# jwr1995/Conv-TasNet

Measured on AMD Instinct MI355X. Metric: utterances/sec (4s, 8kHz, 2-spk) fwd+bwd, higher is better.
Workload: dtype bf16; 1 GPU; paper config train step c2: N=256 L=20 B=256 H=512 P=3 X=8 R=4 gLN non-causal relu-mask, 2 spk, 4 s @ 8 kHz, fwd+PIT loss+bwd+clip+Adam; per_gpu_batch=32, global_batch=32, samples=32000, frames=3199, parallelism=dp1, hip_graph=False

## Files before the change

### conv-tasnet_amd/csrc/ctn_capi_codec.hip

```cpp
#include "ctn_capi_util.h"
#include "ctn_codec.h"

using namespace ctn;


static int codec_check(const ctn_codec_desc* d, bool need_b) {
  if (!d) return fail(CTN_ERR_ARG, "null descriptor");
  if (d->M < 1 || d->T < d->L || d->L < 2 || d->L > 32)
    return fail(CTN_ERR_UNSUPPORTED, "M=%d T=%d L=%d (need T >= L, 2 <= L <= 32)", d->M, d->T, d->L);
  const int S = d->L / 2;
  if (d->K != (d->T - d->L) / S + 1) return fail(CTN_ERR_ARG, "K=%d != (T-L)/(L/2)+1", d->K);
  if (d->Kp != ctn_padded_frames(d->K)) return fail(CTN_ERR_ARG, "Kp=%d != padded(K)", d->Kp);
  const int cg = d->N / 8;
  if (d->N % 8 || cg > 64 || (cg & (cg - 1)))
    return fail(CTN_ERR_UNSUPPORTED, "N=%d: need N/8 a power of two <= 64", d->N);
  if (need_b && (d->B % 8 || d->B < 8)) return fail(CTN_ERR_UNSUPPORTED, "B=%d must be a multiple of 8", d->B);
  if (d->C < 1 || d->C > 16) return fail(CTN_ERR_UNSUPPORTED, "C=%d outside 1..16", d->C);
  if (d->mask_type < 0 || d->mask_type > 2) return fail(CTN_ERR_ARG, "mask_type %d", d->mask_type);
  if (d->dtype != CTN_DTYPE_F32 && d->dtype != CTN_DTYPE_BF16) return fail(CTN_ERR_ARG, "dtype %d", d->dtype);
  return CTN_OK;
}

static CodecArgs codec_args(const ctn_codec_desc* d) {
  CodecArgs a{};
// ... 80 lines not shown
  if (!wb) return CTN_OK;
  const void* wbp = wb;
  if (dt == BF16) {
    CTN_HIP(launch_prep_weight(dt, wb, d->B, d->N, Ly.wbs, nullptr, s));
    wbp = Ly.wbs;
  }
  GemmRows g{};
  g.g = Rows{d->M, d->K, d->Kp}; g.Kred = d->N; g.Nout = d->B; g.norm = NORM_CLN;
  g.A = w_rows; g.lda = d->N;
  g.aop.kind = OP_NORM; g.aop.norm = NORM_CLN; g.aop.stats = a.cln_stats; g.aop.gamma = gamma0; g.aop.beta = beta0;
  g.W = wbp; g.ldw = d->N;
  g.epi = EPI_STORE; g.C = x0; g.ldc = d->B;
  CTN_HIP(launch_gemm_rows(dt, g, s));
  return CTN_OK;
}

extern "C" int ctn_encoder_backward(const ctn_codec_desc* d, const float* mixture, const float* U,
                                    const float* gamma0, const float* beta0, const float* wb, const void* w_rows,
                                    const float* cln_stats, const void* g_w_rows, const void* g_x0, float* gU,
                                    float* ggamma0, float* gbeta0, float* gwb, void* ws, size_t ws_bytes,
                                    void* stream) {
  int rc = codec_check(d, g_x0 != nullptr);
  if (rc) return rc;
  if (!mixture || !w_rows || !gU) return fail(CTN_ERR_ARG, "null pointer");
  if (g_x0 && (!wb || !gamma0 || !beta0 || !cln_stats || !ggamma0 || !gbeta0 || !gwb))
    return fail(CTN_ERR_ARG, "bottleneck backward needs wb/gamma0/beta0/stats and their gradient outputs");
  const EncLayout Ly = enc_layout(d, 1, ws);
  if (!ws || ws_bytes < Ly.bytes) return fail(CTN_ERR_WORKSPACE, "workspace %zu < %zu", ws_bytes, Ly.bytes);
  hipStream_t s = (hipStream_t)stream;
  const DType dt = d->dtype == CTN_DTYPE_BF16 ? BF16 : F32;
  const Rows rg{d->M, d->K, d->Kp};
  CodecArgs a = codec_args(d);
  a.mixture = mixture; a.U = U; a.w_rows = const_cast<void*>(w_rows);
  a.cln_stats = const_cast<float2*>(reinterpret_cast<const float2*>(cln_stats));
  a.gamma0 = gamma0; a.gwdec = g_w_rows; a.gpre = Ly.gpre; a.gpre_bf = Ly.gpre_bf;
  SlabBatch sb{};
  if (g_x0) {
    CTN_HIP(launch_prep_weight(dt, wb, d->B, d->N, nullptr, Ly.wbt, s));
    GemmRows g{};
    g.g = rg; g.Kred = d->B; g.Nout = d->N;
    g.A = g_x0; g.lda = d->B; g.W = Ly.wbt; g.ldw = d->B;
    g.epi = EPI_STORE; g.C = Ly.gcln; g.ldc = d->N;
    CTN_HIP(launch_gemm_rows(dt, g, s));
    GemmCols gc{};
    gc.g = rg; gc.P = d->B; gc.Q = d->N;
    gc.A = g_x0; gc.lda = d->B;
    gc.B = w_rows; gc.ldb = d->N;
    gc.bop.kind = OP_NORM; gc.bop.norm = NORM_CLN; gc.bop.stats = a.cln_stats; gc.bop.gamma = gamma0; gc.bop.beta = beta0;
    gc.Cpart = Ly.cpartB; gc.nchunks = Ly.chunksB;
    CTN_HIP(launch_gemm_cols(dt, gc, s));
    a.gcln = Ly.gcln;
    a.col_slab = Ly.colE;
    sb.d[sb.nd++] = SlabDesc{Ly.cpartB, gwb, Ly.chunksB, d->B * d->N, d->B * d->N};
    sb.d[sb.nd++] = SlabDesc{Ly.colE, ggamma0, Ly.rowblocks, d->N, 2 * d->N};
    sb.d[sb.nd++] = SlabDesc{Ly.colE + d->N, gbeta0, Ly.rowblocks, d->N, 2 * d->N};
  }
  CTN_HIP(launch_enc_bwd_rows(dt, a, s));
  const bool cols = Ly.gpre_bf != nullptr;
  if (cols) {
    a.Lp = Ly.Lp;
    CTN_HIP(launch_frames_bf16(a, mixture, 1, Ly.xfr, s));
    GemmCols gu = du_gemm(d, Ly.Lp);
    gu.A = Ly.gpre_bf; gu.lda = d->N; gu.B = Ly.xfr; gu.ldb = Ly.Lp;
    gu.Cpart = Ly.cpartU; gu.nchunks = Ly.chunksU;
    CTN_HIP(launch_gemm_cols(dt, gu, s));
    sb.d[sb.nd++] = SlabDesc{Ly.cpartU, Ly.Lp == d->L ? gU : Ly.tmpU, Ly.chunksU, d->N * Ly.Lp, d->N * Ly.Lp};
  } else {
    CodecArgs fo = a;
    fo.col_slab = Ly.slabU;
    CTN_HIP(launch_frame_outer(dt, 0, fo, s));
    sb.d[sb.nd++] = SlabDesc{Ly.slabU, gU, Ly.nU, d->N * d->L, d->N * d->L};
  }
  CTN_HIP(launch_slab_reduce(sb, Ly.srtmp, s));
  if (cols && Ly.Lp != d->L) CTN_HIP(launch_unpad_cols(Ly.tmpU, d->N, Ly.Lp, d->L, gU, s));
  return CTN_OK;
}

namespace {
bool dv_cols(const ctn_codec_desc* d) {
  const char* e = getenv("CTN_DV_COLS");
  if (e && atoi(e) == 0) return false;
  return codec_dec_mfma(d->dtype == CTN_DTYPE_BF16 ? BF16 : F32, codec_args(d));
}
GemmCols dv_gemm(const ctn_codec_desc* d, int Lp) {
  GemmCols g{};
  g.g = Rows{d->M, d->K * d->C, d->Kp * d->C};
  g.P = Lp; g.Q = d->N;
  return g;
}
struct DecLayout {
  void *wms, *wmt, *gscore, *srcb, *gfr;
  float *frames, *slabV, *cpartM, *cpartV, *srtmp;
  int nV, chunksM, chunksV, Lp;
  size_t bytes;
};
DecLayout dec_layout(const ctn_codec_desc* d, int backward, bool with_mask_conv, void* ws) {
  DecLayout L{};
  Carver c(ws);
  const size_t es = esize(d->dtype);
  const long rows = (long)d->M * d->Kp;
  const int CN = d->C * d->N;
  if (!backward) {
    if (with_mask_conv && d->dtype == CTN_DTYPE_BF16) L.wms = c.take<void>((size_t)CN * d->B * es);
    L.frames = c.take<float>((size_t)d->M * d->C * d->Kp * d->L * sizeof(float));
  } else {
    CodecArgs a = codec_args(d);
    if (dv_cols(d)) {
      L.Lp = (d->L + 7) & ~7;
      L.srcb = c.take<void>((size_t)rows * d->C * d->N * es);
      L.gfr = c.take<void>((size_t)rows * d->C * L.Lp * es);
      L.chunksV = gemm_cols_default_chunks(dv_gemm(d, L.Lp));
      L.cpartV = c.take<float>((size_t)L.chunksV * L.Lp * d->N * sizeof(float));
    } else {
      L.nV = frame_outer_chunks(a, d->C);
      L.slabV = c.take<float>((size_t)L.nV * d->N * d->L * sizeof(float));
    }
    if (with_mask_conv) {
      L.wmt = c.take<void>((size_t)CN * d->B * es);
      L.gscore = c.take<void>((size_t)rows * CN * es);
      GemmCols gc{};
      gc.g = Rows{d->M, d->K, d->Kp}; gc.P = CN; gc.Q = d->B;
      L.chunksM = gemm_cols_default_chunks(gc);
      L.cpartM = c.take<float>((size_t)L.chunksM * CN * d->B * sizeof(float));
    }
    L.srtmp = c.take<float>((sr_tmp(L.nV > L.chunksV ? L.nV : L.chunksV, (long)d->N * d->L) +
                             sr_tmp(L.chunksM, (long)CN * d->B)) * sizeof(float));
  }
  L.bytes = c.off + 256;
  return L;
}
}

extern "C" size_t ctn_decoder_workspace_bytes(const ctn_codec_desc* d, int backward) {
  if (codec_check(d, d && d->mask_type != CTN_MASK_IDENTITY) != CTN_OK) return 0;
  return dec_layout(d, backward, d->mask_type != CTN_MASK_IDENTITY, nullptr).bytes;
}

extern "C" int ctn_decoder_forward(const ctn_codec_desc* d, const void* x_last, const void* w_rows,
                                   const float* wm, const float* V, void* score, float* est, void* ws,
                                   size_t ws_bytes, void* stream) {
  int rc = codec_check(d, wm != nullptr);
  if (rc) return rc;
  if (!x_last || !w_rows || !V || !est) return fail(CTN_ERR_ARG, "null pointer");
  if ((wm == nullptr) != (d->mask_type == CTN_MASK_IDENTITY))
    return fail(CTN_ERR_ARG, "wm == NULL exactly when mask_type == CTN_MASK_IDENTITY (standalone Decoder)");
  if (wm && !score) return fail(CTN_ERR_ARG, "score output required with the mask conv");
  const DecLayout Ly = dec_layout(d, 0, wm != nullptr, ws);
  if (!ws || ws_bytes < Ly.bytes) return fail(CTN_ERR_WORKSPACE, "workspace %zu < %zu", ws_bytes, Ly.bytes);
  hipStream_t s = (hipStream_t)stream;
  const DType dt = d->dtype == CTN_DTYPE_BF16 ? BF16 : F32;
  const int CN = d->C * d->N;
  const void* sc = x_last;
  if (wm) {
    const void* wmp = wm;
    if (dt == BF16) {
      CTN_HIP(launch_prep_weight(dt, wm, CN, d->B, Ly.wms, nullptr, s));
      wmp = Ly.wms;
    }
    GemmRows g{};
    g.g = Rows{d->M, d->K, d->Kp}; g.Kred = d->B; g.Nout = CN;
    g.A = x_last; g.lda = d->B; g.W = wmp; g.ldw = d->B;
    g.epi = EPI_STORE; g.C = score; g.ldc = CN;
    CTN_HIP(launch_gemm_rows(dt, g, s));
    sc = score;
  }
  CodecArgs a = codec_args(d);
  a.w_rows = const_cast<void*>(w_rows); a.score = sc; a.V = V; a.frames = Ly.frames; a.est = est;
  CTN_HIP(launch_dec_fwd(dt, a, s));
  return CTN_OK;
}

extern "C" int ctn_decoder_backward(const ctn_codec_desc* d, const void* x_last, const void* w_rows,
                                    const float* wm, const float* V, const void* score, const float* g_est,
                                    void* g_x_last, void* g_w_rows, float* gwm, float* gV, void* ws,
                                    size_t ws_bytes, void* stream) {
  int rc = codec_check(d, wm != nullptr);
  if (rc) return rc;
  if (!x_last || !w_rows || !V || !g_est || !g_x_last || !g_w_rows || !gV) return fail(CTN_ERR_ARG, "null pointer");
  if ((wm == nullptr) != (d->mask_type == CTN_MASK_IDENTITY))
    return fail(CTN_ERR_ARG, "wm == NULL exactly when mask_type == CTN_MASK_IDENTITY (standalone Decoder)");
  if (wm && (!score || !gwm)) return fail(CTN_ERR_ARG, "score and gwm required with the mask conv");
  const DecLayout Ly = dec_layout(d, 1, wm != nullptr, ws);
  if (!ws || ws_bytes < Ly.bytes) return fail(CTN_ERR_WORKSPACE, "workspace %zu < %zu", ws_bytes, Ly.bytes);
  hipStream_t s = (hipStream_t)stream;
  const DType dt = d->dtype == CTN_DTYPE_BF16 ? BF16 : F32;
  const Rows rg{d->M, d->K, d->Kp};
  const int CN = d->C * d->N;
  CodecArgs a = codec_args(d);
  a.w_rows = const_cast<void*>(w_rows); a.score = wm ? score : x_last; a.V = V; a.gest = g_est;
  a.gscore = wm ? Ly.gscore : g_x_last; a.gwdec_out = g_w_rows;
  const bool cols = Ly.srcb != nullptr;
  if (cols) { a.src_out = Ly.srcb; a.gfr_out = Ly.gfr; a.Lp = Ly.Lp; }
  CTN_HIP(launch_dec_bwd(dt, a, s));
  SlabBatch sb{};
  if (cols) {
    CTN_HIP(launch_dec_gframes(a, s));
    GemmCols gv = dv_gemm(d, Ly.Lp);
    gv.A = Ly.gfr; gv.lda = Ly.Lp; gv.B = Ly.srcb; gv.ldb = d->N;
    gv.Cpart = Ly.cpartV; gv.nchunks = Ly.chunksV;
    CTN_HIP(launch_gemm_cols(dt, gv, s));
    sb.d[sb.nd++] = SlabDesc{Ly.cpartV, gV, Ly.chunksV, d->N * d->L, Ly.Lp * d->N};
  } else {
    CodecArgs fo = a;
    fo.col_slab = Ly.slabV;
    CTN_HIP(launch_frame_outer(dt, 1, fo, s));
    sb.d[sb.nd++] = SlabDesc{Ly.slabV, gV, Ly.nV, d->N * d->L, d->N * d->L};
  }
  if (wm) {
    CTN_HIP(launch_prep_weight(dt, wm, CN, d->B, nullptr, Ly.wmt, s));
    GemmRows g{};
    g.g = rg; g.Kred = CN; g.Nout = d->B;
    g.A = Ly.gscore; g.lda = CN; g.W = Ly.wmt; g.ldw = CN;
    g.epi = EPI_STORE; g.C = g_x_last; g.ldc = d->B;
    CTN_HIP(launch_gemm_rows(dt, g, s));
    GemmCols gc{};
    gc.g = rg; gc.P = CN; gc.Q = d->B;
    gc.A = Ly.gscore; gc.lda = CN; gc.B = x_last; gc.ldb = d->B;
    gc.Cpart = Ly.cpartM; gc.nchunks = Ly.chunksM;
    CTN_HIP(launch_gemm_cols(dt, gc, s));
    sb.d[sb.nd++] = SlabDesc{Ly.cpartM, gwm, Ly.chunksM, CN * d->B, CN * d->B};
  }
  CTN_HIP(launch_slab_reduce(sb, Ly.srtmp, s));
  return CTN_OK;
}
```

### conv-tasnet_amd/csrc/ctn_codec.h

```cpp
#pragma once
#include "ctn_kernels.h"

namespace ctn {

struct CodecArgs {
  int M, T, K, Kp, N, L, S, C;
  int mask_type;
  const float* mixture;
  const float* U;
  const float* V;
  void* w_rows;
  float2* cln_stats;
  const float* gamma0;
  const void* gcln;
  const void* gwdec;
  float* gpre;
  float* col_slab;
  const void* score;
  float* frames;
  float* est;
  const float* gest;
  void* gscore;
  void* gwdec_out;
  void* src_out = nullptr;
  void* gfr_out = nullptr;
  int Lp = 0;
  void* gpre_bf = nullptr;
};
bool codec_dec_mfma(DType dt, const CodecArgs& a);
hipError_t launch_dec_gframes(const CodecArgs& a, hipStream_t s);
hipError_t launch_frames_bf16(const CodecArgs& a, const float* sig, int C, void* out, hipStream_t s);
hipError_t launch_unpad_cols(const float* tmp, int N, int Lp, int L, float* out, hipStream_t s);

hipError_t launch_enc_fwd(DType dt, const CodecArgs& a, hipStream_t s);
hipError_t launch_enc_bwd_rows(DType dt, const CodecArgs& a, hipStream_t s);
int frame_outer_chunks(const CodecArgs& a, int C);
hipError_t launch_frame_outer(DType dt, int mode, const CodecArgs& a, hipStream_t s);
hipError_t launch_dec_fwd(DType dt, const CodecArgs& a, hipStream_t s);
hipError_t launch_dec_bwd(DType dt, const CodecArgs& a, hipStream_t s);

struct PitArgs {
  int M, C, T;
  const float* src;
  const float* est;
  const int64_t* lengths;
  double* slab;
  int chunks;
  float* max_snr;
  int64_t* best;
  float* coef;
  float* loss;
  const float* g_loss;
  const float* g_maxsnr;
  float* gest;
  float* est_inplace;
  float* reordered;
  double* msd;
  int nperm;
  int perms[24][4];
};
int pit_nv(int C);
hipError_t launch_pit_forward(const PitArgs& a, hipStream_t s);
hipError_t launch_pit_backward(const PitArgs& a, hipStream_t s);

}
```

### conv-tasnet_amd/csrc/ctn_codec.hip

```cpp
#include <stdlib.h>

#include "ctn_common.h"
#include "ctn_codec.h"

namespace ctn {

constexpr int EN_RPB = 128;

template <typename T>
__global__ __launch_bounds__(256) void enc_fwd_kernel(CodecArgs a) {
  extern __shared__ __attribute__((aligned(16))) float sm[];
  const int N = a.N, L = a.L, S = a.S, cg = N / 8;
  int nrl = 256 / cg;
  if (nrl > EN_RPB) nrl = EN_RPB;
  const int tid = threadIdx.x, c = tid % cg, rl = tid / cg;
  const bool act = rl < nrl;
  const int K = a.K, Kp = a.Kp;
  const int row0 = blockIdx.x * EN_RPB, m = row0 / Kp, k0 = row0 - m * Kp;
  float* Ut = sm;
  float* xs = sm + L * N;
  const int nsamp = (EN_RPB - 1) * S + L;
  for (int i = tid; i < L * N; i += 256) {
    const int l = i / N, n = i % N;
    Ut[i] = a.U[n * L + l];
// ... 363 lines not shown
    for (int c = 0; c < CM; ++c)
      if (c < C) mx = fmaxf(mx, x[c]);
#pragma unroll
    for (int c = 0; c < CM; ++c)
      if (c < C) {
        x[c] = __expf(x[c] - mx);
        den += x[c];
      }
#pragma unroll
    for (int c = 0; c < CM; ++c)
      if (c < C) x[c] /= den;
  } else if (mask_type == 0) {
#pragma unroll
    for (int c = 0; c < CM; ++c) x[c] = x[c] > 0.f ? x[c] : 0.f;
  }
}

template <int KBN, int CM>
__global__ __launch_bounds__(256) void dec_fwd_mfma_kernel(CodecArgs a) {
  constexpr int N = KBN * 32;
  __shared__ v4u bfrag[2 * KBN * 64];
  const int lane = threadIdx.x & 63, lg = lane >> 4, wv = threadIdx.x >> 6;
  const int L = a.L, C = a.C, K = a.K, Kp = a.Kp;
  for (int i = threadIdx.x; i < 2 * KBN * 64; i += 256) {
    const int ln = i & 63, kb = (i >> 6) % KBN, nb = i / (64 * KBN), l = nb * 16 + (ln & 15);
    float f[8] = {0, 0, 0, 0, 0, 0, 0, 0};
    if (l < L) Vec8<float>::load(a.V + (size_t)l * N + kb * 32 + 8 * (ln >> 4), f);
    bfrag[i] = pack_bf16x8v(f);
  }
  __syncthreads();
  const int lr = lane & 15;
  const bf16raw* w = reinterpret_cast<const bf16raw*>(a.w_rows);
  const bf16raw* sc = reinterpret_cast<const bf16raw*>(a.score);
  const long nblk = (long)a.M * Kp / 16;
  for (long blk = (long)blockIdx.x * DM_WAVES + wv; blk < nblk; blk += (long)gridDim.x * DM_WAVES) {
    const long r0 = blk * 16;
    const int m = (int)(r0 / Kp), k0 = (int)(r0 - (long)m * Kp);
    if (k0 >= K) continue;
    const long r = r0 + lr;
    f32x4_t acc[CM][2];
#pragma unroll
    for (int c = 0; c < CM; ++c) acc[c][0] = acc[c][1] = f32x4_t{0.f, 0.f, 0.f, 0.f};
#pragma unroll
    for (int kb = 0; kb < KBN; ++kb) {
      const int ch = kb * 32 + 8 * lg;
      float wf[8], sf[CM][8];
      unpack_bf16x8(ldg16(w + r * N + ch), wf);
#pragma unroll
      for (int c = 0; c < CM; ++c)
        if (c < C) unpack_bf16x8(ldg16(sc + r * (long)(C * N) + (long)c * N + ch), sf[c]);
#pragma unroll
      for (int e = 0; e < 8; ++e) {
        float x[CM];
#pragma unroll
        for (int c = 0; c < CM; ++c) x[c] = c < C ? sf[c][e] : 0.f;
        dm_act<CM>(a.mask_type, C, x);
#pragma unroll
        for (int c = 0; c < CM; ++c) sf[c][e] = wf[e] * x[c];
      }
#pragma unroll
      for (int c = 0; c < CM; ++c)
        if (c < C) {
          const bf16x8_t af = __builtin_bit_cast(bf16x8_t, pack_bf16x8v(sf[c]));
          const v4u b0 = bfrag[kb * 64 + lane], b1 = bfrag[(KBN + kb) * 64 + lane];
          acc[c][0] = __builtin_amdgcn_mfma_f32_16x16x32_bf16(af, __builtin_bit_cast(bf16x8_t, b0), acc[c][0], 0, 0, 0);
          acc[c][1] = __builtin_amdgcn_mfma_f32_16x16x32_bf16(af, __builtin_bit_cast(bf16x8_t, b1), acc[c][1], 0, 0, 0);
        }
    }
#pragma unroll
    for (int c = 0; c < CM; ++c)
      if (c < C)
#pragma unroll
        for (int nb = 0; nb < 2; ++nb) {
          const int l = nb * 16 + lr;
          if (l >= L) continue;
          float* f = a.frames + (((size_t)m * C + c) * Kp + k0) * L + l;
#pragma unroll
          for (int i = 0; i < 4; ++i)
            if (k0 + 4 * lg + i < K) f[(size_t)(4 * lg + i) * L] = acc[c][nb][i];
        }
  }
}

template <int NBN, int CM>
__global__ __launch_bounds__(256) void dec_bwd_mfma_kernel(CodecArgs a) {
  constexpr int N = NBN * 16;
  static_assert(NBN % 2 == 0, "two channel blocks per round");
  __shared__ v4u afrag[NBN * 64];
  constexpr int TS = 36;
  __shared__ __attribute__((aligned(16))) float gtile[DM_WAVES * CM * 16 * TS];
  const int lane = threadIdx.x & 63, lr = lane & 15, lg = lane >> 4, wv = threadIdx.x >> 6;
  const int L = a.L, C = a.C, S = a.S, K = a.K, Kp = a.Kp;
  for (int i = threadIdx.x; i < NBN * 64; i += 256) {
    const int ln = i & 63, nb = i >> 6;
    float f[8];
#pragma unroll
    for (int j = 0; j < 8; ++j) {
      const int l = 8 * (ln >> 4) + j;
      f[j] = l < L ? a.V[(size_t)l * N + nb * 16 + (ln & 15)] : 0.f;
    }
    afrag[i] = pack_bf16x8v(f);
  }
  __syncthreads();
  const bf16raw* w = reinterpret_cast<const bf16raw*>(a.w_rows);
  const bf16raw* sc = reinterpret_cast<const bf16raw*>(a.score);
  bf16raw* gsc = reinterpret_cast<bf16raw*>(a.gscore);
  bf16raw* gw = reinterpret_cast<bf16raw*>(a.gwdec_out);
  const long nblk = (long)a.M * Kp / 16;
  typedef uint32_t v2u __attribute__((ext_vector_type(2)));
  for (long blk = (long)blockIdx.x * DM_WAVES + wv; blk < nblk; blk += (long)gridDim.x * DM_WAVES) {
    const long r0 = blk * 16;
    const int m = (int)(r0 / Kp), k0 = (int)(r0 - (long)m * Kp);
    v4u gb[CM];
    {
      const int k = k0 + lr;
#pragma unroll
      for (int c = 0; c < CM; ++c) {
        float f[8] = {0, 0, 0, 0, 0, 0, 0, 0};
        if (c < C && k < K) {
          const float* g = a.gest + ((size_t)m * C + c) * a.T + (long)k * S;
#pragma unroll
          for (int j = 0; j < 8; ++j) {
            const int l = 8 * lg + j;
            if (l < L && (long)k * S + l < a.T) f[j] = g[l];
          }
        }
        gb[c] = pack_bf16x8v(f);
      }
    }
    float* tile = gtile + wv * (CM * 16 * TS);
    const int er = lane >> 2, en = 8 * (lane & 3);
#pragma unroll 1
    for (int nb = 0; nb < NBN; nb += 2) {
      const long r = r0 + er;
      const int n0 = nb * 16 + en;
      const v4u wraw = ldg16(w + r * N + n0);
      v4u sraw[CM];
#pragma unroll
      for (int c = 0; c < CM; ++c) sraw[c] = c < C ? ldg16(sc + r * (long)(C * N) + (long)c * N + n0) : v4u{0u, 0u, 0u, 0u};
#pragma unroll
      for (int h = 0; h < 2; ++h)
#pragma unroll
        for (int c = 0; c < CM; ++c)
          if (c < C) {
            const f32x4_t g = __builtin_amdgcn_mfma_f32_16x16x32_bf16(
                __builtin_bit_cast(bf16x8_t, afrag[(nb + h) * 64 + lane]), __builtin_bit_cast(bf16x8_t, gb[c]),
                f32x4_t{0.f, 0.f, 0.f, 0.f}, 0, 0, 0);
            *reinterpret_cast<float4*>(tile + (c * 16 + lr) * TS + h * 16 + 4 * lg) = float4{g[0], g[1], g[2], g[3]};
          }
      asm volatile("s_waitcnt lgkmcnt(0)" ::: "memory");
      float wf[8], sv[CM][8], gs[CM][8];
      unpack_bf16x8(wraw, wf);
#pragma unroll
      for (int c = 0; c < CM; ++c)
        if (c < C) {
          unpack_bf16x8(sraw[c], sv[c]);
          const float4 g0 = *reinterpret_cast<const float4*>(tile + (c * 16 + er) * TS + en);
          const float4 g1 = *reinterpret_cast<const float4*>(tile + (c * 16 + er) * TS + en + 4);
          gs[c][0] = g0.x; gs[c][1] = g0.y; gs[c][2] = g0.z; gs[c][3] = g0.w;
          gs[c][4] = g1.x; gs[c][5] = g1.y; gs[c][6] = g1.z; gs[c][7] = g1.w;
        }
      float gwv[8], go[CM][8], srcv[CM][8];
#pragma unroll
      for (int i = 0; i < 8; ++i) {
        float s[CM], act[CM];
#pragma unroll
        for (int c = 0; c < CM; ++c) {
          s[c] = c < C ? sv[c][i] : 0.f;
          act[c] = s[c];
        }
        dm_act<CM>(a.mask_type, C, act);
#pragma unroll
        for (int c = 0; c < CM; ++c) srcv[c][i] = wf[i] * act[c];
        float gwe = 0.f, dot = 0.f, ga[CM];
#pragma unroll
        for (int c = 0; c < CM; ++c) {
          ga[c] = 0.f;
          if (c < C) {
            gwe += gs[c][i] * act[c];
            ga[c] = gs[c][i] * wf[i];
            dot += ga[c] * act[c];
          }
        }
        gwv[i] = gwe;
#pragma unroll
        for (int c = 0; c < CM; ++c)
          if (c < C) {
            float g = ga[c];
            if (a.mask_type == 0 && !(s[c] > 0.f)) g = 0.f;
            if (a.mask_type == 1) g = act[c] * (ga[c] - dot);
            go[c][i] = g;
          }
      }
#pragma unroll
      for (int c = 0; c < CM; ++c)
        if (c < C) stg16(gsc + r * (long)(C * N) + (long)c * N + n0, pack_bf16x8v(go[c]));
      stg16(gw + r * N + n0, pack_bf16x8v(gwv));
      if (a.src_out) {
        bf16raw* so = reinterpret_cast<bf16raw*>(a.src_out);
#pragma unroll
        for (int c = 0; c < CM; ++c)
          if (c < C) stg16(so + r * (long)(C * N) + (long)c * N + n0, pack_bf16x8v(srcv[c]));
      }
      asm volatile("s_waitcnt lgkmcnt(0)" ::: "memory");
    }
  }
}

__global__ __launch_bounds__(256) void frames_bf16_kernel(CodecArgs a, const float* sig, int C, bf16raw* out) {
  const long n = (long)a.M * a.Kp * C;
  for (long i = blockIdx.x * 256L + threadIdx.x; i < n; i += (long)gridDim.x * 256) {
    const int c = (int)(i % C);
    const long r = i / C;
    const int m = (int)(r / a.Kp), k = (int)(r % a.Kp);
    const float* g = sig + ((size_t)m * C + c) * a.T + (long)k * a.S;
    bf16raw* o = out + i * a.Lp;
    for (int l0 = 0; l0 < a.Lp; l0 += 8) {
      float f[8];
#pragma unroll
      for (int j = 0; j < 8; ++j) {
        const int l = l0 + j;
        f[j] = (k < a.K && l < a.L && (long)k * a.S + l < a.T) ? g[l] : 0.f;
      }
      stg16(o + l0, pack_bf16x8v(f));
    }
  }
}

template <int NBN>
__global__ __launch_bounds__(256) void enc_fwd_mfma_kernel(CodecArgs a) {
  constexpr int N = NBN * 16, NR = NBN / 2;
  constexpr int TS = 36, KKM = 8;
  __shared__ float afr[NBN * KKM * 64];
  __shared__ __attribute__((aligned(16))) float tiles[DM_WAVES * 16 * TS];
  const int lane = threadIdx.x & 63, lr = lane & 15, lg = lane >> 4, wv = threadIdx.x >> 6;
  const int L = a.L, S = a.S, K = a.K, Kp = a.Kp, KK = (L + 3) / 4;
  for (int i = threadIdx.x; i < NBN * KKM * 64; i += 256) {
    const int ln = i & 63, kk = (i >> 6) % KKM, nb = i / (64 * KKM), l = 4 * kk + (ln >> 4);
    afr[i] = l < L ? a.U[(size_t)(nb * 16 + (ln & 15)) * L + l] : 0.f;
  }
  __syncthreads();
  bf16raw* w = reinterpret_cast<bf16raw*>(a.w_rows);
  float* tile = tiles + wv * 16 * TS;
  const int er = lane >> 2, en = 8 * (lane & 3);
  const long nblk = (long)a.M * Kp / 16;
  for (long blk = (long)blockIdx.x * DM_WAVES + wv; blk < nblk; blk += (long)gridDim.x * DM_WAVES) {
    const long r0 = blk * 16;
    const int m = (int)(r0 / Kp), k0 = (int)(r0 - (long)m * Kp);
    float fb[KKM];
    {
      const int k = k0 + lr;
      const float* x = a.mixture + (size_t)m * a.T + (long)k * S;
#pragma unroll
      for (int kk = 0; kk < KKM; ++kk) {
        const int l = 4 * kk + lg;
        fb[kk] = (kk < KK && k < K && l < L && (long)k * S + l < a.T) ? x[l] : 0.f;
      }
    }
    const int k = k0 + er;
    const bool valid = k < K;
    float v[NR][8];
#pragma unroll
    for (int rd = 0; rd < NR; ++rd) {
#pragma unroll
      for (int h = 0; h < 2; ++h) {
        f32x4_t g = f32x4_t{0.f, 0.f, 0.f, 0.f};
#pragma unroll
        for (int kk = 0; kk < KKM; ++kk)
          if (kk < KK) g = __builtin_amdgcn_mfma_f32_16x16x4f32(afr[((2 * rd + h) * KKM + kk) * 64 + lane], fb[kk], g, 0, 0, 0);
        *reinterpret_cast<float4*>(tile + lr * TS + h * 16 + 4 * lg) = float4{g[0], g[1], g[2], g[3]};
      }
      asm volatile("s_waitcnt lgkmcnt(0)" ::: "memory");
      const float4 g0 = *reinterpret_cast<const float4*>(tile + er * TS + en);
      const float4 g1 = *reinterpret_cast<const float4*>(tile + er * TS + en + 4);
      const float t[8] = {g0.x, g0.y, g0.z, g0.w, g1.x, g1.y, g1.z, g1.w};
#pragma unroll
      for (int e = 0; e < 8; ++e) v[rd][e] = valid ? (t[e] > 0.f ? t[e] : 0.f) : 0.f;
      stg16(w + (size_t)(r0 + er) * N + rd * 32 + en, pack_bf16x8v(v[rd]));
      asm volatile("s_waitcnt lgkmcnt(0)" ::: "memory");
    }
    if (a.cln_stats) {
      float sm = 0.f;
#pragma unroll
      for (int rd = 0; rd < NR; ++rd)
#pragma unroll
        for (int e = 0; e < 8; ++e) sm += v[rd][e];
      sm += dpp_f<0xB1, 0xF>(sm);
      sm += dpp_f<0x4E, 0xF>(sm);
      const float mean = sm / (float)N;
      float q = 0.f;
#pragma unroll
      for (int rd = 0; rd < NR; ++rd)
#pragma unroll
        for (int e = 0; e < 8; ++e) q += (v[rd][e] - mean) * (v[rd][e] - mean);
      q += dpp_f<0xB1, 0xF>(q);
      q += dpp_f<0x4E, 0xF>(q);
      if ((lane & 3) == 0) {
        const float rstd = 1.0f / sqrtf(q / (float)N + 1e-8f);
        a.cln_stats[r0 + er] = valid ? make_float2(mean, rstd) : make_float2(0.f, 1.f);
      }
    }
  }
}

bool codec_dec_mfma(DType dt, const CodecArgs& a);
static bool dec_mfma(DType dt, const CodecArgs& a) { return codec_dec_mfma(dt, a); }
bool codec_dec_mfma(DType dt, const CodecArgs& a) {
  const char* e = getenv("CTN_DEC_MFMA");
  if (e && atoi(e) == 0) return false;
  return dt == BF16 && (a.N == 256 || a.N == 512) && a.L <= 32 && a.C <= 4;
}
static unsigned dm_grid(const CodecArgs& a) {
  const long waves = (long)a.M * a.Kp / 16;
  long wgs = (waves + DM_WAVES - 1) / DM_WAVES;
  return (unsigned)(wgs < 1024 ? wgs : 1024);
}

static bool codec_ok(const CodecArgs& a) {
  return a.N % 8 == 0 && a.N / 8 <= 64 && ((a.N / 8) & (a.N / 8 - 1)) == 0 && a.L >= 1 && a.L <= 32 &&
         a.S >= 1 && a.C >= 1 && a.C <= 16 && a.Kp % EN_RPB == 0;
}

hipError_t launch_enc_fwd(DType dt, const CodecArgs& a, hipStream_t s) {
  if (!codec_ok(a)) return hipErrorInvalidValue;
  const size_t lds = ((size_t)a.L * a.N + (EN_RPB - 1) * a.S + a.L) * sizeof(float);
  const dim3 g((unsigned)((long)a.M * a.Kp / EN_RPB)), b(256);
  const char* e = getenv("CTN_ENC_MFMA");
  const bool mf = dt == BF16 && (!e || atoi(e) != 0) && (a.N == 256 || a.N == 512) && a.L <= 32;
  if (mf && a.N == 256) hipLaunchKernelGGL(enc_fwd_mfma_kernel<16>, dim3(dm_grid(a)), b, 0, s, a);
  else if (mf) hipLaunchKernelGGL(enc_fwd_mfma_kernel<32>, dim3(dm_grid(a)), b, 0, s, a);
  else if (dt == BF16) hipLaunchKernelGGL(enc_fwd_kernel<bf16raw>, g, b, lds, s, a);
  else hipLaunchKernelGGL(enc_fwd_kernel<float>, g, b, lds, s, a);
  return hipGetLastError();
}

hipError_t launch_enc_bwd_rows(DType dt, const CodecArgs& a, hipStream_t s) {
  if (!codec_ok(a)) return hipErrorInvalidValue;
  const dim3 g((unsigned)((long)a.M * a.Kp / EN_RPB)), b(256);
  if (dt == BF16) hipLaunchKernelGGL(enc_bwd_rows_kernel<bf16raw>, g, b, 0, s, a);
  else hipLaunchKernelGGL(enc_bwd_rows_kernel<float>, g, b, 0, s, a);
  return hipGetLastError();
}

int frame_outer_chunks(const CodecArgs& a, int C) {
  const int n = a.M * (a.Kp / fo_rows(C));
  return n < FO_WGS ? n : FO_WGS;
}

hipError_t launch_frame_outer(DType dt, int mode, const CodecArgs& a, hipStream_t s) {
  if (!codec_ok(a) || a.Kp % FO_R || a.N > 512 || a.L > FO_LMAX) return hipErrorInvalidValue;
  const int C = mode == 0 ? 1 : a.C;
  const int fr = fo_rows(C);
  const size_t lds = ((size_t)fr * C * a.N + (size_t)C * (fr * a.S + a.L)) * sizeof(float);
  if (lds > 160 * 1024) return hipErrorInvalidValue;
  const dim3 g(frame_outer_chunks(a, C)), b(256);
#define CTN_FO(T_, M_)                                                                                          \
  if (C > 8) hipLaunchKernelGGL((frame_outer_kernel<T_, M_, 0, 16>), g, b, lds, s, a);                       \
  else if (C > 4) hipLaunchKernelGGL((frame_outer_kernel<T_, M_, 0, 8>), g, b, lds, s, a);                   \
  else if (a.L == 20) hipLaunchKernelGGL((frame_outer_kernel<T_, M_, 20>), g, b, lds, s, a);                  \
  else if (a.L == 16) hipLaunchKernelGGL((frame_outer_kernel<T_, M_, 16>), g, b, lds, s, a);                  \
  else hipLaunchKernelGGL((frame_outer_kernel<T_, M_, 0>), g, b, lds, s, a);
  if (mode == 0) {
    if (dt == BF16) { CTN_FO(bf16raw, 0) } else { CTN_FO(float, 0) }
  } else {
    if (dt == BF16) { CTN_FO(bf16raw, 1) } else { CTN_FO(float, 1) }
  }
#undef CTN_FO
  return hipGetLastError();
}

static int dec_rpb(const CodecArgs& a) {
  const size_t budget = 64 * 1024 - (((size_t)a.N * a.L + 3) & ~(size_t)3) * 4;
  int rpb = 32;
  while (rpb > 1 && (size_t)rpb * a.C * a.N * 4 > budget) rpb >>= 1;
  return rpb;
}

hipError_t launch_dec_fwd(DType dt, const CodecArgs& a, hipStream_t s) {
  if (!codec_ok(a)) return hipErrorInvalidValue;
  const int rpb = dec_rpb(a);
  const size_t lds = (((size_t)a.N * a.L + 3) & ~(size_t)3) * 4 + (size_t)rpb * a.C * a.N * 4;
  const dim3 g((unsigned)((long)a.M * a.Kp / rpb)), b(256);
  if (dec_mfma(dt, a)) {
#define CTN_DFM(KBN_)                                                                                    \
    switch (a.C) {                                                                                     \
      case 1: hipLaunchKernelGGL((dec_fwd_mfma_kernel<KBN_, 1>), dim3(dm_grid(a)), b, 0, s, a); break; \
      case 2: hipLaunchKernelGGL((dec_fwd_mfma_kernel<KBN_, 2>), dim3(dm_grid(a)), b, 0, s, a); break; \
      case 3: hipLaunchKernelGGL((dec_fwd_mfma_kernel<KBN_, 3>), dim3(dm_grid(a)), b, 0, s, a); break; \
      default: hipLaunchKernelGGL((dec_fwd_mfma_kernel<KBN_, 4>), dim3(dm_grid(a)), b, 0, s, a); break; \
    }
    if (a.N == 256) { CTN_DFM(8) } else { CTN_DFM(16) }
#undef CTN_DFM
  } else if (a.C > 8) {
    if (dt == BF16) hipLaunchKernelGGL((dec_fwd_kernel<bf16raw, 16>), g, b, lds, s, a, rpb);
    else hipLaunchKernelGGL((dec_fwd_kernel<float, 16>), g, b, lds, s, a, rpb);
  } else if (a.C > 4) {
    if (dt == BF16) hipLaunchKernelGGL((dec_fwd_kernel<bf16raw, 8>), g, b, lds, s, a, rpb);
    else hipLaunchKernelGGL((dec_fwd_kernel<float, 8>), g, b, lds, s, a, rpb);
  } else if (dt == BF16) hipLaunchKernelGGL(dec_fwd_kernel<bf16raw>, g, b, lds, s, a, rpb);
  else hipLaunchKernelGGL(dec_fwd_kernel<float>, g, b, lds, s, a, rpb);
  hipError_t e = hipGetLastError();
  if (e != hipSuccess) return e;
  long total = (long)a.M * a.C * a.T;
  int gb = (int)((total + 255) / 256);
  if (gb > 4096) gb = 4096;
  hipLaunchKernelGGL(ola_fwd_kernel, dim3(gb), dim3(256), 0, s, a);
  return hipGetLastError();
}

hipError_t launch_frames_bf16(const CodecArgs& a, const float* sig, int C, void* out, hipStream_t s) {
  if (!out || !sig || a.Lp < a.L || a.Lp % 8 || C < 1) return hipErrorInvalidValue;
  const long n = (long)a.M * a.Kp * C;
  long g = (n + 255) / 256;
  hipLaunchKernelGGL(frames_bf16_kernel, dim3((unsigned)(g < 4096 ? g : 4096)), dim3(256), 0, s, a, sig, C,
                     reinterpret_cast<bf16raw*>(out));
  return hipGetLastError();
}
hipError_t launch_dec_gframes(const CodecArgs& a, hipStream_t s) {
  return launch_frames_bf16(a, a.gest, a.C, a.gfr_out, s);
}

__global__ __launch_bounds__(256) void unpad_cols_kernel(const float* tmp, int N, int Lp, int L, float* out) {
  const int i = blockIdx.x * 256 + threadIdx.x;
  if (i < N * L) out[i] = tmp[(i / L) * Lp + i % L];
}
hipError_t launch_unpad_cols(const float* tmp, int N, int Lp, int L, float* out, hipStream_t s) {
  hipLaunchKernelGGL(unpad_cols_kernel, dim3((N * L + 255) / 256), dim3(256), 0, s, tmp, N, Lp, L, out);
  return hipGetLastError();
}

hipError_t launch_dec_bwd(DType dt, const CodecArgs& a, hipStream_t s) {
  if (!codec_ok(a)) return hipErrorInvalidValue;
  const int rpb = 32;
  const size_t lds = (((size_t)a.N * a.L + 3) & ~(size_t)3) * 4 + (size_t)rpb * a.C * a.L * 4;
  const dim3 g((unsigned)((long)a.M * a.Kp / rpb)), b(256);
  if (dec_mfma(dt, a)) {
#define CTN_DBM(NBN_)                                                                                     \
    switch (a.C) {                                                                                      \
      case 1: hipLaunchKernelGGL((dec_bwd_mfma_kernel<NBN_, 1>), dim3(dm_grid(a)), b, 0, s, a); break;  \
      case 2: hipLaunchKernelGGL((dec_bwd_mfma_kernel<NBN_, 2>), dim3(dm_grid(a)), b, 0, s, a); break;  \
      case 3: hipLaunchKernelGGL((dec_bwd_mfma_kernel<NBN_, 3>), dim3(dm_grid(a)), b, 0, s, a); break;  \
      default: hipLaunchKernelGGL((dec_bwd_mfma_kernel<NBN_, 4>), dim3(dm_grid(a)), b, 0, s, a); break; \
    }
    if (a.N == 256) { CTN_DBM(16) } else { CTN_DBM(32) }
#undef CTN_DBM
  } else if (a.C > 8) {
    if (dt == BF16) hipLaunchKernelGGL((dec_bwd_kernel<bf16raw, 16>), g, b, lds, s, a, rpb);
    else hipLaunchKernelGGL((dec_bwd_kernel<float, 16>), g, b, lds, s, a, rpb);
  } else if (a.C > 4) {
    if (dt == BF16) hipLaunchKernelGGL((dec_bwd_kernel<bf16raw, 8>), g, b, lds, s, a, rpb);
    else hipLaunchKernelGGL((dec_bwd_kernel<float, 8>), g, b, lds, s, a, rpb);
  } else if (dt == BF16) hipLaunchKernelGGL(dec_bwd_kernel<bf16raw>, g, b, lds, s, a, rpb);
  else hipLaunchKernelGGL(dec_bwd_kernel<float>, g, b, lds, s, a, rpb);
  return hipGetLastError();
}

}
```

Baseline: 2335 utterances/sec.

## Fuse decoder basis-weight gradient GEMM into MFMA decoder backward kernel

The decoder backward kernel now accumulates the decoder basis gradient (gV) directly with MFMA, using LDS-transposed fragments of the gradient frames and source estimates. This removes the separate frame-packing kernel, the bf16 source and gradient-frame intermediates written to global memory, and the column GEMM. The kernel also switches to a contiguous per-block row range with a fixed CU-sized grid, prefetches the next rows' loads through a two-slot register ring, and specializes on mask type and channel count at compile time. The cost is higher register and LDS pressure and fewer blocks, which could lower occupancy. The gV partial slab now shares workspace with the mask-conv partials and is reduced early to make that sharing safe.

```diff
diff --git a/conv-tasnet_amd/csrc/ctn_capi_codec.hip b/conv-tasnet_amd/csrc/ctn_capi_codec.hip
--- a/conv-tasnet_amd/csrc/ctn_capi_codec.hip
+++ b/conv-tasnet_amd/csrc/ctn_capi_codec.hip
@@ -186,16 +186,10 @@
   if (e && atoi(e) == 0) return false;
   return codec_dec_mfma(d->dtype == CTN_DTYPE_BF16 ? BF16 : F32, codec_args(d));
 }
-GemmCols dv_gemm(const ctn_codec_desc* d, int Lp) {
-  GemmCols g{};
-  g.g = Rows{d->M, d->K * d->C, d->Kp * d->C};
-  g.P = Lp; g.Q = d->N;
-  return g;
-}
 struct DecLayout {
-  void *wms, *wmt, *gscore, *srcb, *gfr;
+  void *wms, *wmt, *gscore;
   float *frames, *slabV, *cpartM, *cpartV, *srtmp;
-  int nV, chunksM, chunksV, Lp;
+  int nV, chunksM, chunksV;
   size_t bytes;
 };
 DecLayout dec_layout(const ctn_codec_desc* d, int backward, bool with_mask_conv, void* ws) {
@@ -209,12 +203,12 @@
     L.frames = c.take<float>((size_t)d->M * d->C * d->Kp * d->L * sizeof(float));
   } else {
     CodecArgs a = codec_args(d);
-    if (dv_cols(d)) {
-      L.Lp = (d->L + 7) & ~7;
-      L.srcb = c.take<void>((size_t)rows * d->C * d->N * es);
-      L.gfr = c.take<void>((size_t)rows * d->C * L.Lp * es);
-      L.chunksV = gemm_cols_default_chunks(dv_gemm(d, L.Lp));
-      L.cpartV = c.take<float>((size_t)L.chunksV * L.Lp * d->N * sizeof(float));
+    const bool cols = dv_cols(d);
+    size_t bytesV = 0;
+    if (cols) {
+      L.chunksV = dec_bwd_mfma_grid(a);
+      bytesV = (size_t)L.chunksV * d->L * d->N * sizeof(float);
+      if (!with_mask_conv) L.cpartV = c.take<float>(bytesV);
     } else {
       L.nV = frame_outer_chunks(a, d->C);
       L.slabV = c.take<float>((size_t)L.nV * d->N * d->L * sizeof(float));
@@ -225,7 +219,9 @@
       GemmCols gc{};
       gc.g = Rows{d->M, d->K, d->Kp}; gc.P = CN; gc.Q = d->B;
       L.chunksM = gemm_cols_default_chunks(gc);
-      L.cpartM = c.take<float>((size_t)L.chunksM * CN * d->B * sizeof(float));
+      const size_t bytesM = (size_t)L.chunksM * CN * d->B * sizeof(float);
+      L.cpartM = c.take<float>(bytesM > bytesV ? bytesM : bytesV);
+      if (cols) L.cpartV = L.cpartM;
     }
     L.srtmp = c.take<float>((sr_tmp(L.nV > L.chunksV ? L.nV : L.chunksV, (long)d->N * d->L) +
                              sr_tmp(L.chunksM, (long)CN * d->B)) * sizeof(float));
@@ -293,17 +289,16 @@
   CodecArgs a = codec_args(d);
   a.w_rows = const_cast<void*>(w_rows); a.score = wm ? score : x_last; a.V = V; a.gest = g_est;
   a.gscore = wm ? Ly.gscore : g_x_last; a.gwdec_out = g_w_rows;
-  const bool cols = Ly.srcb != nullptr;
-  if (cols) { a.src_out = Ly.srcb; a.gfr_out = Ly.gfr; a.Lp = Ly.Lp; }
+  const bool cols = Ly.cpartV != nullptr;
+  if (cols) a.col_slab = Ly.cpartV;
   CTN_HIP(launch_dec_bwd(dt, a, s));
   SlabBatch sb{};
   if (cols) {
-    CTN_HIP(launch_dec_gframes(a, s));
-    GemmCols gv = dv_gemm(d, Ly.Lp);
-    gv.A = Ly.gfr; gv.lda = Ly.Lp; gv.B = Ly.srcb; gv.ldb = d->N;
-    gv.Cpart = Ly.cpartV; gv.nchunks = Ly.chunksV;
-    CTN_HIP(launch_gemm_cols(dt, gv, s));
-    sb.d[sb.nd++] = SlabDesc{Ly.cpartV, gV, Ly.chunksV, d->N * d->L, Ly.Lp * d->N};
+    sb.d[sb.nd++] = SlabDesc{Ly.cpartV, gV, Ly.chunksV, d->N * d->L, d->N * d->L};
+    if (wm) {
+      CTN_HIP(launch_slab_reduce(sb, Ly.srtmp, s));
+      sb.nd = 0;
+    }
   } else {
     CodecArgs fo = a;
     fo.col_slab = Ly.slabV;
diff --git a/conv-tasnet_amd/csrc/ctn_codec.h b/conv-tasnet_amd/csrc/ctn_codec.h
--- a/conv-tasnet_amd/csrc/ctn_codec.h
+++ b/conv-tasnet_amd/csrc/ctn_codec.h
@@ -22,13 +22,11 @@
   const float* gest;
   void* gscore;
   void* gwdec_out;
-  void* src_out = nullptr;
-  void* gfr_out = nullptr;
   int Lp = 0;
   void* gpre_bf = nullptr;
 };
 bool codec_dec_mfma(DType dt, const CodecArgs& a);
-hipError_t launch_dec_gframes(const CodecArgs& a, hipStream_t s);
+int dec_bwd_mfma_grid(const CodecArgs& a);
 hipError_t launch_frames_bf16(const CodecArgs& a, const float* sig, int C, void* out, hipStream_t s);
 hipError_t launch_unpad_cols(const float* tmp, int N, int Lp, int L, float* out, hipStream_t s);
 
diff --git a/conv-tasnet_amd/csrc/ctn_codec.hip b/conv-tasnet_amd/csrc/ctn_codec.hip
--- a/conv-tasnet_amd/csrc/ctn_codec.hip
+++ b/conv-tasnet_amd/csrc/ctn_codec.hip
@@ -469,15 +469,28 @@
   }
 }
 
-template <int NBN, int CM>
+CTN_DEV bf16x8_t dm_tr_frag(const bf16raw* img, int row0, int col0, int lane) {
+  const int lr = lane & 15, lg = lane >> 4;
+  const bf16raw* p = img + (row0 + 8 * lg + (lr >> 2)) * 32 + col0 + 4 * (lr & 3);
+  const s16x4_t lo = __builtin_amdgcn_ds_read_tr16_b64_v4i16((__attribute__((address_space(3))) s16x4_t*)(p));
+  const s16x4_t hi = __builtin_amdgcn_ds_read_tr16_b64_v4i16((__attribute__((address_space(3))) s16x4_t*)(p + 4 * 32));
+  return bf16x8_t{lo[0], lo[1], lo[2], lo[3], hi[0], hi[1], hi[2], hi[3]};
+}
+
+template <int NBN, int CM, bool DV>
 __global__ __launch_bounds__(256) void dec_bwd_mfma_kernel(CodecArgs a) {
-  constexpr int N = NBN * 16;
-  static_assert(NBN % 2 == 0, "two channel blocks per round");
+  constexpr int N = NBN * 16, NW = N / DM_WAVES, NRW = NW / 32;
+  static_assert(NRW >= 2 && NRW % 2 == 0, "the two-slot ring needs an even number of rounds");
+  constexpr int CP = (CM + 1) & ~1;
   __shared__ v4u afrag[NBN * 64];
   constexpr int TS = 36;
   __shared__ __attribute__((aligned(16))) float gtile[DM_WAVES * CM * 16 * TS];
+  __shared__ __attribute__((aligned(16))) bf16raw dvimg[DV ? DM_WAVES * 2 * CP * 16 * 32 : 8];
   const int lane = threadIdx.x & 63, lr = lane & 15, lg = lane >> 4, wv = threadIdx.x >> 6;
-  const int L = a.L, C = a.C, S = a.S, K = a.K, Kp = a.Kp;
+  const int L = a.L, S = a.S, K = a.K, Kp = a.Kp;
+  constexpr int C = CM;
+  if constexpr (DV)
+    for (int i = threadIdx.x; i < DM_WAVES * 2 * CP * 16 * 32 / 8; i += 256) stg16(dvimg + 8 * i, v4u{0u, 0u, 0u, 0u});
   for (int i = threadIdx.x; i < NBN * 64; i += 256) {
     const int ln = i & 63, nb = i >> 6;
     float f[8];
@@ -493,38 +506,82 @@
   const bf16raw* sc = reinterpret_cast<const bf16raw*>(a.score);
   bf16raw* gsc = reinterpret_cast<bf16raw*>(a.gscore);
   bf16raw* gw = reinterpret_cast<bf16raw*>(a.gwdec_out);
-  const long nblk = (long)a.M * Kp / 16;
-  typedef uint32_t v2u __attribute__((ext_vector_type(2)));
-  for (long blk = (long)blockIdx.x * DM_WAVES + wv; blk < nblk; blk += (long)gridDim.x * DM_WAVES) {
-    const long r0 = blk * 16;
-    const int m = (int)(r0 / Kp), k0 = (int)(r0 - (long)m * Kp);
+  const int nblk = (int)((long)a.M * Kp / 16);
+  const int b0 = (int)((long)nblk * blockIdx.x / gridDim.x), b1 = (int)((long)nblk * (blockIdx.x + 1) / gridDim.x);
+  float* tile = gtile + wv * (CM * 16 * TS);
+  bf16raw* gimg = dvimg + (DV ? wv * (2 * CP * 16 * 32) : 0);
+  bf16raw* simg = gimg + (DV ? CP * 16 * 32 : 0);
+  const int er = lane >> 2, en = 8 * (lane & 3);
+  const int nw0 = wv * NW;
+  f32x4_t dv[2][NW / 16];
+#pragma unroll
+  for (int lb = 0; lb < 2; ++lb)
+#pragma unroll
+    for (int cb = 0; cb < NW / 16; ++cb) dv[lb][cb] = f32x4_t{0.f, 0.f, 0.f, 0.f};
+  struct RowSet { v4u w, s[CM]; };
+  auto rload = [&](RowSet& R, int blk, int rd) __attribute__((always_inline)) {
+    const long r = (long)blk * 16 + er;
+    const int n0 = nw0 + rd * 32 + en;
+    R.w = ldg16(w + r * N + n0);
+#pragma unroll
+    for (int c = 0; c < CM; ++c) R.s[c] = c < C ? ldg16(sc + r * (long)(C * N) + (long)c * N + n0) : v4u{0u, 0u, 0u, 0u};
+  };
+  auto gload = [&](float (&f)[CM][8], int blk) __attribute__((always_inline)) {
+    const long r0 = (long)blk * 16;
+    const int m = (int)(r0 / Kp), k = (int)(r0 - (long)m * Kp) + lr;
+#pragma unroll
+    for (int c = 0; c < CM; ++c) {
+      const float* g = a.gest + ((size_t)m * C + c) * a.T;
+#pragma unroll
+      for (int j = 0; j < 8; ++j) {
+        const long t = (long)k * S + 8 * lg + j;
+        f[c][j] = g[t < a.T ? t : a.T - 1];
+      }
+    }
+  };
+  auto gzero = [&](float (&f)[CM][8], int blk) __attribute__((always_inline)) {
+    const int k = (int)(((long)blk * 16) % Kp) + lr;
+#pragma unroll
+    for (int j = 0; j < 8; ++j) {
+      const int l = 8 * lg + j;
+      const bool in = k < K && l < L && (long)k * S + l < a.T;
+#pragma unroll
+      for (int c = 0; c < CM; ++c) f[c][j] = in ? f[c][j] : 0.f;
+    }
+  };
+  RowSet R[2];
+  float gn[CM][8];
+  if (b0 < b1) {
+    rload(R[0], b0, 0);
+    gload(gn, b0);
+  }
+  auto run = [&](auto mtc) __attribute__((always_inline)) {
+  constexpr int MT = decltype(mtc)::value;
+  for (int blk = b0; blk < b1; ++blk) {
+    const long r0 = (long)blk * 16;
+    const int nxt = blk + 1 < b1 ? blk + 1 : blk;
     v4u gb[CM];
-    {
-      const int k = k0 + lr;
-#pragma unroll
-      for (int c = 0; c < CM; ++c) {
-        float f[8] = {0, 0, 0, 0, 0, 0, 0, 0};
-        if (c < C && k < K) {
-          const float* g = a.gest + ((size_t)m * C + c) * a.T + (long)k * S;
-#pragma unroll
-          for (int j = 0; j < 8; ++j) {
-            const int l = 8 * lg + j;
-            if (l < L && (long)k * S + l < a.T) f[j] = g[l];
-          }
-        }
-        gb[c] = pack_bf16x8v(f);
-      }
-    }
-    float* tile = gtile + wv * (CM * 16 * TS);
-    const int er = lane >> 2, en = 8 * (lane & 3);
-#pragma unroll 1
-    for (int nb = 0; nb < NBN; nb += 2) {
+    gzero(gn, blk);
+#pragma unroll
+    for (int c = 0; c < CM; ++c) gb[c] = pack_bf16x8v(gn[c]);
+    gload(gn, nxt);
+    bf16x8_t ga[2][CP / 2];
+    if constexpr (DV) {
+#pragma unroll
+      for (int c = 0; c < CM; ++c)
+        if (c < C) stg16(gimg + (c * 16 + lr) * 32 + 8 * lg, gb[c]);
+      asm volatile("s_waitcnt lgkmcnt(0)" ::: "memory");
+#pragma unroll
+      for (int lb = 0; lb < 2; ++lb)
+#pragma unroll
+        for (int pr = 0; pr < CP / 2; ++pr) ga[lb][pr] = dm_tr_frag(gimg, 32 * pr, 16 * lb, lane);
+    }
+    static_for<NRW>([&](auto rdc) __attribute__((always_inline)) {
+      constexpr int rd = decltype(rdc)::value;
+      if constexpr (rd + 1 < NRW) rload(R[(rd + 1) & 1], blk, rd + 1);
+      else rload(R[0], nxt, 0);
       const long r = r0 + er;
-      const int n0 = nb * 16 + en;
-      const v4u wraw = ldg16(w + r * N + n0);
-      v4u sraw[CM];
-#pragma unroll
-      for (int c = 0; c < CM; ++c) sraw[c] = c < C ? ldg16(sc + r * (long)(C * N) + (long)c * N + n0) : v4u{0u, 0u, 0u, 0u};
+      const int n0 = nw0 + rd * 32 + en, nb = (nw0 + rd * 32) / 16;
 #pragma unroll
       for (int h = 0; h < 2; ++h)
 #pragma unroll
@@ -536,6 +593,13 @@
             *reinterpret_cast<float4*>(tile + (c * 16 + lr) * TS + h * 16 + 4 * lg) = float4{g[0], g[1], g[2], g[3]};
           }
       asm volatile("s_waitcnt lgkmcnt(0)" ::: "memory");
+      v4u wraw = R[rd & 1].w, sraw[CM];
+      asm volatile("" : "+v"(wraw));
+#pragma unroll
+      for (int c = 0; c < CM; ++c) {
+        sraw[c] = R[rd & 1].s[c];
+        asm volatile("" : "+v"(sraw[c]));
+      }
       float wf[8], sv[CM][8], gs[CM][8];
       unpack_bf16x8(wraw, wf);
 #pragma unroll
@@ -550,13 +614,14 @@
       float gwv[8], go[CM][8], srcv[CM][8];
 #pragma unroll
       for (int i = 0; i < 8; ++i) {
+#pragma clang fp contract(off)
         float s[CM], act[CM];
 #pragma unroll
         for (int c = 0; c < CM; ++c) {
           s[c] = c < C ? sv[c][i] : 0.f;
           act[c] = s[c];
         }
-        dm_act<CM>(a.mask_type, C, act);
+        dm_act<CM>(MT, C, act);
 #pragma unroll
         for (int c = 0; c < CM; ++c) srcv[c][i] = wf[i] * act[c];
         float gwe = 0.f, dot = 0.f, ga[CM];
@@ -564,9 +629,9 @@
         for (int c = 0; c < CM; ++c) {
           ga[c] = 0.f;
           if (c < C) {
-            gwe += gs[c][i] * act[c];
+            gwe = __builtin_fmaf(gs[c][i], act[c], gwe);
             ga[c] = gs[c][i] * wf[i];
-            dot += ga[c] * act[c];
+            dot = __builtin_fmaf(ga[c], act[c], dot);
           }
         }
         gwv[i] = gwe;
@@ -574,8 +639,8 @@
         for (int c = 0; c < CM; ++c)
           if (c < C) {
             float g = ga[c];
-            if (a.mask_type == 0 && !(s[c] > 0.f)) g = 0.f;
-            if (a.mask_type == 1) g = act[c] * (ga[c] - dot);
+            if (MT == 0 && !(s[c] > 0.f)) g = 0.f;
+            if (MT == 1) g = act[c] * (ga[c] - dot);
             go[c][i] = g;
           }
       }
@@ -583,14 +648,39 @@
       for (int c = 0; c < CM; ++c)
         if (c < C) stg16(gsc + r * (long)(C * N) + (long)c * N + n0, pack_bf16x8v(go[c]));
       stg16(gw + r * N + n0, pack_bf16x8v(gwv));
-      if (a.src_out) {
-        bf16raw* so = reinterpret_cast<bf16raw*>(a.src_out);
+      if constexpr (DV) {
 #pragma unroll
         for (int c = 0; c < CM; ++c)
-          if (c < C) stg16(so + r * (long)(C * N) + (long)c * N + n0, pack_bf16x8v(srcv[c]));
+          if (c < C) stg16(simg + (c * 16 + er) * 32 + en, pack_bf16x8v(srcv[c]));
+        asm volatile("s_waitcnt lgkmcnt(0)" ::: "memory");
+#pragma unroll
+        for (int h = 0; h < 2; ++h)
+#pragma unroll
+          for (int pr = 0; pr < CP / 2; ++pr) {
+            const bf16x8_t sb = dm_tr_frag(simg, 32 * pr, 16 * h, lane);
+#pragma unroll
+            for (int lb = 0; lb < 2; ++lb)
+              dv[lb][2 * rd + h] = __builtin_amdgcn_mfma_f32_16x16x32_bf16(ga[lb][pr], sb, dv[lb][2 * rd + h], 0, 0, 0);
+          }
       }
       asm volatile("s_waitcnt lgkmcnt(0)" ::: "memory");
-    }
+    });
+  }
+  };
+  if (a.mask_type == 0) run(std::integral_constant<int, 0>{});
+  else if (a.mask_type == 1) run(std::integral_constant<int, 1>{});
+  else run(std::integral_constant<int, 2>{});
+  if constexpr (DV) {
+    float* out = a.col_slab + (size_t)blockIdx.x * N * L;
+#pragma unroll
+    for (int lb = 0; lb < 2; ++lb)
+#pragma unroll
+      for (int cb = 0; cb < NW / 16; ++cb)
+#pragma unroll
+        for (int i = 0; i < 4; ++i) {
+          const int l = lb * 16 + 4 * lg + i;
+          if (l < L) out[(size_t)l * N + nw0 + cb * 16 + lr] = dv[lb][cb][i];
+        }
   }
 }
 
@@ -701,6 +791,21 @@
   const long waves = (long)a.M * a.Kp / 16;
   long wgs = (waves + DM_WAVES - 1) / DM_WAVES;
   return (unsigned)(wgs < 1024 ? wgs : 1024);
+}
+
+static int dm_cus() {
+  static const int cus = [] {
+    int dev = 0, n = 0;
+    if (hipGetDevice(&dev) != hipSuccess ||
+        hipDeviceGetAttribute(&n, hipDeviceAttributeMultiprocessorCount, dev) != hipSuccess || n <= 0)
+      n = 256;
+    return n;
+  }();
+  return cus;
+}
+int dec_bwd_mfma_grid(const CodecArgs& a) {
+  const long nblk = (long)a.M * a.Kp / 16, cap = (a.C <= 2 ? 2L : 1L) * dm_cus(), g = nblk / 4;
+  return (int)(g < 1 ? 1 : (g < cap ? g : cap));
 }
 
 static bool codec_ok(const CodecArgs& a) {
@@ -803,10 +908,6 @@
                      reinterpret_cast<bf16raw*>(out));
   return hipGetLastError();
 }
-hipError_t launch_dec_gframes(const CodecArgs& a, hipStream_t s) {
-  return launch_frames_bf16(a, a.gest, a.C, a.gfr_out, s);
-}
-
 __global__ __launch_bounds__(256) void unpad_cols_kernel(const float* tmp, int N, int Lp, int L, float* out) {
   const int i = blockIdx.x * 256 + threadIdx.x;
   if (i < N * L) out[i] = tmp[(i / L) * Lp + i % L];
@@ -822,14 +923,19 @@
   const size_t lds = (((size_t)a.N * a.L + 3) & ~(size_t)3) * 4 + (size_t)rpb * a.C * a.L * 4;
   const dim3 g((unsigned)((long)a.M * a.Kp / rpb)), b(256);
   if (dec_mfma(dt, a)) {
-#define CTN_DBM(NBN_)                                                                                     \
-    switch (a.C) {                                                                                      \
-      case 1: hipLaunchKernelGGL((dec_bwd_mfma_kernel<NBN_, 1>), dim3(dm_grid(a)), b, 0, s, a); break;  \
-      case 2: hipLaunchKernelGGL((dec_bwd_mfma_kernel<NBN_, 2>), dim3(dm_grid(a)), b, 0, s, a); break;  \
-      case 3: hipLaunchKernelGGL((dec_bwd_mfma_kernel<NBN_, 3>), dim3(dm_grid(a)), b, 0, s, a); break;  \
-      default: hipLaunchKernelGGL((dec_bwd_mfma_kernel<NBN_, 4>), dim3(dm_grid(a)), b, 0, s, a); break; \
+    const dim3 gd(dec_bwd_mfma_grid(a));
+#define CTN_DBM2(NBN_, C_)                                                                    \
+    if (a.col_slab) hipLaunchKernelGGL((dec_bwd_mfma_kernel<NBN_, C_, true>), gd, b, 0, s, a); \
+    else hipLaunchKernelGGL((dec_bwd_mfma_kernel<NBN_, C_, false>), gd, b, 0, s, a);
+#define CTN_DBM(NBN_)                   \
+    switch (a.C) {                      \
+      case 1: CTN_DBM2(NBN_, 1) break;  \
+      case 2: CTN_DBM2(NBN_, 2) break;  \
+      case 3: CTN_DBM2(NBN_, 3) break;  \
+      default: CTN_DBM2(NBN_, 4) break; \
     }
     if (a.N == 256) { CTN_DBM(16) } else { CTN_DBM(32) }
+#undef CTN_DBM2
 #undef CTN_DBM
   } else if (a.C > 8) {
     if (dt == BF16) hipLaunchKernelGGL((dec_bwd_kernel<bf16raw, 16>), g, b, lds, s, a, rpb);
```

Result: no change. 2351 utterances/sec, median of 6 (+0.7%).
